# peteroh23/ModulationDetectionCNN

Hardware: AMD Instinct MI355X
Metric: I/Q frames/sec (2x128, VT-CNN2, batch=2^20) (higher is better)
Workload: dtype bf16; 1 GPU; vtcnn2-c11-bf16-n2^20; topology=vtcnn2, classes=11, frames_per_gpu=1048576, global_batch=1048576, parallelism=batch-shard x1 (no collective), outputs=softmax probabilities f32 + argmax int32, frames_per_forward_call=1048576, full=False

## Files before the change

modulationdetectioncnn_amd/build.py:

```python
from __future__ import annotations

import hashlib
import os
import shutil
import subprocess
import sys
from concurrent.futures import ThreadPoolExecutor

HERE = os.path.dirname(os.path.abspath(__file__))
ROOT = os.path.dirname(HERE)
CSRC = os.path.join(HERE, "csrc")
OBJ = os.path.join(HERE, "csrc", "build")
LIB = os.path.join(HERE, "libmdc.so")
ARCH = "gfx950"
VERSION_SCRIPT = os.path.join(CSRC, "libmdc.map")
VARIANTS = {"product": (OBJ, LIB, ()),
            "alternates": (os.path.join(HERE, "csrc", "build_alt"), os.path.join(HERE, "libmdc_alt.so"), ("-DMDC_ALTERNATES",))}

CXXFLAGS = ["-O3", "-std=c++17", "-fPIC", f"--offload-arch={ARCH}", "-I", os.path.join(ROOT, "include"),
            "-I", CSRC, "-Wall", "-Wno-unused-function", "-pthread",
            "-fvisibility=hidden", "-fvisibility-inlines-hidden"]


def _hipcc() -> str:
    exe = shutil.which("hipcc") or "/opt/rocm/bin/hipcc"
    if not os.path.exists(exe):
        raise RuntimeError("hipcc not found: libmdc.so cannot be built")
    return exe


def sources():
    return sorted(os.path.join(CSRC, f) for f in os.listdir(CSRC) if f.endswith(".hip"))


def _newer(a: str, deps) -> bool:
    if not os.path.exists(a):
        return False
    t = os.path.getmtime(a)
    return all(os.path.getmtime(d) <= t for d in deps)


def flag_key(extra_flags=()) -> str:
    return hashlib.sha256(" ".join([*CXXFLAGS, *extra_flags]).encode()).hexdigest()


def build(force: bool = False, verbose: bool = False, extra_flags=(), variant: str = "product") -> str:
    obj_dir, lib_path, vflags = VARIANTS[variant]
    extra_flags = (*vflags, *extra_flags)
    os.makedirs(obj_dir, exist_ok=True)
    stamp = os.path.join(obj_dir, "flags.stamp")
    hipcc = _hipcc()
    headers = [os.path.join(CSRC, f) for f in os.listdir(CSRC) if f.endswith(".h")] + [os.path.join(ROOT, "include", "mdc.h")]
    key = flag_key(extra_flags)
    if not (os.path.exists(stamp) and open(stamp).read().strip() == key):
        force = True
    jobs = []
    objs = []
    for src in sources():
        obj = os.path.join(obj_dir, os.path.basename(src)[:-4] + ".o")
        objs.append(obj)
        if force or not _newer(obj, [src] + headers):
            jobs.append((src, obj))
# ... 39 lines not shown
```

modulationdetectioncnn_amd/csrc/mdc_api.hip:

```cpp
#include "mdc_internal.h"

#include <cstdlib>
#include <cstring>
#include <exception>
#include <mutex>
#include <new>

namespace mdc {

static thread_local char g_err[512] = "";

void set_error(const char* fmt, ...) {
    va_list ap;
    va_start(ap, fmt);
    vsnprintf(g_err, sizeof(g_err), fmt, ap);
    va_end(ap);
}

int upload(mdc_model* m, int idx, const void* host, size_t bytes) {
    if (m->d_pack[idx]) {
        (void)hipFree(m->d_pack[idx]);
        m->d_pack[idx] = nullptr;
    }
    MDC_HIP(hipMalloc(&m->d_pack[idx], bytes));
// ... 96 lines not shown
        if (std::strncmp(prop.gcnArchName, "gfx950", 6) != 0) {
            set_error("device %d is %s; libmdc.so carries gfx950 (MI355X) code only", device, prop.gcnArchName);
            return MDC_ENODEV;
        }
        mdc_model* m = new (std::nothrow) mdc_model();
        if (!m) { set_error("out of host memory"); return MDC_ENOMEM; }
        m->topo = *topo;
        m->device = device;
#ifdef MDC_ALTERNATES
        {
            auto flag = [](const char* name, int when) { const char* e = getenv(name); return e && atoi(e) == when; };
            if (flag("MDC_CONV_SCHED", 0)) m->alt |= kAltConvHipcc;
            if (flag("MDC_DENSE1_PHASED", 0)) m->alt |= kAltDense1Simple;
            if (flag("MDC_DEP_F32_MFMA", 1)) m->alt |= kAltDepF32Mfma;
            if (flag("MDC_D1_FUSED_HEAD", 0)) m->alt |= kAltSeparateHead;
            if (const char* e = getenv("MDC_DEP_RING")) m->alt_ring = atoi(e);
        }
#endif
        int rc = MDC_ENOMEM;
        try { rc = layer_layout(m); } catch (...) { delete m; throw; }
        if (rc != MDC_OK) { delete m; return rc; }
        *out = m;
        return MDC_OK;
    });
}

int mdc_num_layers(const mdc_model* m) {
    if (!m) { set_error("null model"); return MDC_EINVAL; }
    return m->nlayers;
}
// ... 341 lines not shown
```

modulationdetectioncnn_amd/csrc/mdc_internal.h:

```cpp
#pragma once
#include <hip/hip_runtime.h>
#include <cstdarg>
#include <cstdint>
#include <cstdio>
#include <exception>
#include <mutex>
#include <new>
#include <string>
#include <type_traits>
#include <vector>

#include "mdc.h"

namespace mdc {

void set_error(const char* fmt, ...);

template <class Fn>
inline int guarded(const char* what, Fn&& fn) noexcept {
    try {
        return fn();
    } catch (const std::bad_alloc&) {
        set_error("%s: out of host memory", what);
        return MDC_ENOMEM;
// ... 47 lines not shown
};
template <bool CHECK> using HopOrNf = typename std::conditional<CHECK, NfArgs, long>::type;
__device__ __forceinline__ long hop_of(long h) { return h; }
__device__ __forceinline__ long hop_of(const NfArgs&) { return 256; }
__device__ __forceinline__ NfArgs nf_of(long) { return NfArgs{nullptr, nullptr, 0}; }
__device__ __forceinline__ NfArgs nf_of(const NfArgs& a) { return a; }
constexpr unsigned kNfInfBits = 0x7F800000u;
__device__ __forceinline__ unsigned nf_absbits_max4(const float4 v) {
    return max(max(__float_as_uint(v.x) & 0x7FFFFFFFu, __float_as_uint(v.y) & 0x7FFFFFFFu),
               max(__float_as_uint(v.z) & 0x7FFFFFFFu, __float_as_uint(v.w) & 0x7FFFFFFFu));
}

enum { kAltConvHipcc = 1,
       kAltDense1Simple = 2,
       kAltDepF32Mfma = 4,
       kAltSeparateHead = 8 };

struct ProfSlot {
    const char* name;
    std::vector<hipEvent_t> ev;
    double total_ms = 0;
    int64_t launches = 0;
};

}

struct mdc_model {
    mdc_topology topo{};
    int device = 0;
    int dtype = MDC_F32;
    bool finalized = false;
// ... 60 lines not shown
                    int64_t chunk_frames);
int predict_host_iq_norm(mdc_model* m, const void* iq_host, int format, int64_t n, int64_t hop, float level, int flags, float* probs_host,
                         int32_t* labels_host, mdc_iq_window_stats64* stats_host, int64_t chunk_frames);
void host_ctx_free(mdc_model* m);

int deployed_pack(mdc_model* m);
int deployed_f32m_pack(mdc_model* m);
int deployed_f32m_forward(const mdc_model* m, const float* x, int64_t n, float* probs, int32_t* labels, float* tap_dense, hipStream_t s);
int deployed_f32m_forward_iq_u8(const mdc_model* m, const uint8_t* iq, int64_t n, long hop2, float scale, float* probs, int32_t* labels, hipStream_t s);
int deployed_bf16_pack(mdc_model* m);
int deployed_bf16_forward(const mdc_model* m, const float* x, int64_t n, float* probs, int32_t* labels, hipStream_t s);
int deployed_bf16_forward_iq_u8(const mdc_model* m, const uint8_t* iq, int64_t n, int64_t hop, float scale, float* probs, int32_t* labels, hipStream_t s);
int deployed_q612_pack(mdc_model* m);
int deployed_q612_forward(const mdc_model* m, const void* x, int x_is_q, int64_t n, int32_t* dense, int32_t* labels, hipStream_t s);
int vtcnn2_fp8_pack(mdc_model* m);
int vtcnn2_fp8_conv(const mdc_model* m, const float* x, int64_t n, void* feat, hipStream_t s, long hop2 = 0, float scale = 0.f);
int confusion_launch(const int32_t* truth, const int32_t* pred, const int32_t* bin, int64_t n, int classes, int bins, int64_t* counts,
                     int64_t* bad, hipStream_t s);
int crossentropy_launch(const float* probs, const int32_t* truth, int64_t n, int classes, double* loss_sum, int64_t* bad, hipStream_t s);
int iq_u8_launch(const uint8_t* iq, int64_t n, int64_t hop, float scale, float* x, hipStream_t s);
int iq_norm_check(const char* who, int64_t hop, float level, int flags);
int iq_norm_launch(const uint8_t* iq, int64_t n, int64_t hop, float level, int flags, float* x, mdc_iq_window_stats* stats, hipStream_t s);
int iq_pair_bytes(int format);
int iq_format_check(const char* who, int format, int64_t hop);
int iq_fmt_windows_launch(const void* iq, int format, int64_t n, int64_t hop, float scale, float* x, hipStream_t s);
int iq_fmt_norm_launch(const void* iq, int format, int64_t n, int64_t hop, float level, int flags, float* x, mdc_iq_window_stats64* stats,
                       hipStream_t s);
int nonfinite_launch(const float* x, int64_t n, uint8_t* flags, int64_t* count, float* probs, int32_t* labels, int classes, bool poison,
                     hipStream_t s);
int deployed_forward(const mdc_model* m, const float* x, int64_t n, float* probs, int32_t* labels,
                     float* tap, int tap_kind, hipStream_t s);
// ... 19 lines not shown
```

modulationdetectioncnn_amd/csrc/vtcnn2.hip:

```cpp
#include "dense_chain_common.h"

#include <algorithm>
#include <cmath>

namespace mdc {

namespace {

__device__ __forceinline__ void glds16(const void* g, void* lds_wave_base) {
    const unsigned l = (unsigned)(size_t)(__attribute__((address_space(3))) unsigned char*)lds_wave_base;
    asm volatile("global_load_lds_dwordx4 %0, off" ::"v"(g), "{m0}"(l) : "memory");
}
__device__ __forceinline__ void glds_drain_and_barrier() {
    asm volatile("s_waitcnt vmcnt(0)" ::: "memory");
    __syncthreads();
}

constexpr int kChunk = 16;
constexpr int kNChunk = kC1 / kChunk;
constexpr int kWChunkFloats = 2 * 3 * 5 * 4 * 64;
constexpr int kXld = 133;
constexpr int kXinFloats = 4 * 2 * 16 * kXld;
constexpr size_t kConvF32Lds = (2 * kWChunkFloats + kXinFloats) * sizeof(float);

// ... 372 lines not shown
    const int o = r / kW2, w = r % kW2;
    const unsigned v = feat[f * kFeat + feat8_index(w, o)];
    const int e = (int)((v >> 3) & 15u), mant = (int)(v & 7u);
    float mag = e == 0 ? ldexpf((float)mant, -9) : ldexpf(1.f + (float)mant * 0.125f, e - 7);
    if ((v & 0x7Fu) == 0x7Fu) mag = __uint_as_float(0x7FC00000u);
    out[i] = ((v & 0x80u) ? -mag : mag) * unscale;
}

}

void chain_pack_layer(std::vector<float>& dst, const float* w, int k_in, int n_out, int ksteps, int tiles);
int chain_launch(int t1, int nl, const float* x, long n, const float* wpack, int n_out, int relu1, int relu2,
                 float* probs, int* labels, float* tap_logits, float* tap_h1, float* tap_h2, int n1, int n2, hipStream_t s);

int vtcnn2_bf16_pack(mdc_model* m);
int vtcnn2_bf16_conv(const mdc_model* m, const float* x, int64_t n, void* feat, hipStream_t s, long hop2 = 0, float scale = 0.f);
int vtcnn2_bf16_dense1(const mdc_model* m, const void* feat, int64_t n, float* hid, hipStream_t s,
                       bool fuse_head, float* probs, int32_t* labels, bool* fused);

int vtcnn2_pack(mdc_model* m) {
    const float* k1 = m->hk[0].data();
    const float* b1 = m->hb[0].data();
    const float* k2 = m->hk[1].data();
    int rc;
    if ((rc = upload(m, 2, m->hb[1].data(), kC2 * sizeof(float)))) return rc;
    if ((rc = upload(m, 4, m->hb[2].data(), kHid * sizeof(float)))) return rc;
    {
        const int C = m->topo.classes;
        if (C > 16) { set_error("vtcnn2: the HIP head covers up to 16 classes (got %d)", C); return MDC_ENOTSUP; }
        std::vector<float> pk;
        chain_pack_layer(pk, m->hk[3].data(), kHid, C, 64, 1);
// ... 41 lines not shown
    return np * kFeat * feat_elem(m) + np * kHid * sizeof(float);
}

static int vtcnn2_run(const mdc_model* m, const float* x, long hop2, float scale, int64_t n, float* probs, int32_t* labels,
                      float* tap, int tap_kind, void* ws, size_t ws_bytes, hipStream_t s) {
    const size_t need = vtcnn2_workspace_bytes(m, n);
    if (!ws || ws_bytes < need) { set_error("vtcnn2 forward of %lld frames needs %zu workspace bytes (got %zu)", (long long)n, need, ws_bytes); return MDC_EINVAL; }
    if ((reinterpret_cast<uintptr_t>(ws) & 255) != 0) { set_error("workspace must be 256-byte aligned"); return MDC_EINVAL; }
    const size_t fbytes = (((size_t)n + 255) & ~(size_t)255) * kFeat * feat_elem(m);
    void* feat = ws;
    float* hid = reinterpret_cast<float*>(static_cast<char*>(ws) + fbytes);
    const int C = m->topo.classes;
    int rc;
    bool head_done = false;
    if (m->dtype == MDC_BF16 || m->dtype == MDC_FP8) {
        { ProfScope ps(m, 0, s); if ((rc = m->dtype == MDC_FP8 ? vtcnn2_fp8_conv(m, x, n, feat, s, hop2, scale) : vtcnn2_bf16_conv(m, x, n, feat, s, hop2, scale))) return rc; }
        const bool fuse = tap_kind != MDC_TAP_DENSE && tap_kind != MDC_TAP_HIDDEN;
        { ProfScope ps(m, 1, s); if ((rc = vtcnn2_bf16_dense1(m, feat, n, hid, s, fuse, probs, labels, &head_done))) return rc; }
    } else {
        {
            ProfScope ps(m, 0, s);
            const unsigned groups = (unsigned)((n + 63) / 64);
            constexpr long t1 = 128, t3 = 2048, t11 = 8192;
#define MDC_LAUNCH_CONV_F32(U, KP, YS) do { \
                MDC_HIP(hipFuncSetAttribute(reinterpret_cast<const void*>(vt_conv_f32_kernel<U, KP, YS>), hipFuncAttributeMaxDynamicSharedMemorySize, (int)kConvF32Lds)); \
                hipLaunchKernelGGL((vt_conv_f32_kernel<U, KP, YS>), dim3(groups, YS ? kW2 / KP : 1), dim3(256), kConvF32Lds, s, x, (long)n, \
                                   static_cast<const float*>(m->d_pack[0]), static_cast<const float*>(m->d_pack[1]), \
                                   static_cast<const float*>(m->d_pack[2]), static_cast<float*>(feat), hop2 > 0 ? hop2 : 256L, scale); } while (0)
            if (hop2 > 0) {
                if (n <= t1) MDC_LAUNCH_CONV_F32(true, 1, true);
                else if (n <= t3) MDC_LAUNCH_CONV_F32(true, 3, true);
// ... 82 lines not shown
```

modulationdetectioncnn_amd/csrc/vtcnn2_bf16.hip:

```cpp
#include "vtcnn2_bf16_common.h"
#include "vtcnn2_sched_common.h"

#include <cmath>

#include <cstdlib>
#include <cstring>
#include <type_traits>

namespace mdc {

namespace {

#ifdef MDC_ALTERNATES
__global__ __launch_bounds__(256, 1) void vt_conv_bf16_kernel(const float* __restrict__ x, long n,
                                                              const u32x4* __restrict__ wq,
                                                              const u32x2* __restrict__ a1q,
                                                              const float* __restrict__ b2,
                                                              unsigned short* __restrict__ feat) {
    extern __shared__ __attribute__((aligned(16))) unsigned char smem[];
    unsigned* img = reinterpret_cast<unsigned*>(smem);
    float* part = reinterpret_cast<float*>(smem + (size_t)2 * kImgWords * 4);
    const int tid = threadIdx.x, lane = tid & 63;
    const int q = __builtin_amdgcn_readfirstlane(tid >> 6);
    const int nl = lane & 15, g = lane >> 4;
// ... 228 lines not shown
        if ((rc = upload(m, 2, b2s.data(), b2s.size() * sizeof(float)))) return rc;
    }
    m->feat_scale_log2 = -kFeatShift;
    const float* w1 = m->hk[2].data();
    std::vector<unsigned short> w1t((size_t)kHid * kFeat);
    for (int w = 0; w < kW2; ++w)
        for (int o = 0; o < kC2; ++o) {
            const float* src = w1 + (size_t)(o * kW2 + w) * kHid;
            const int kk = feat16_index(w, o);
            for (int nn = 0; nn < kHid; ++nn) w1t[((size_t)(kk >> 6) * kHid + nn) * 64 + (kk & 63)] = f2bf(std::ldexp(src[nn], kFeatShift));
        }
    if ((rc = upload(m, 3, w1t.data(), w1t.size() * 2))) return rc;
    return vtcnn2_bf16_pack_sched(m);
}

int vtcnn2_bf16_conv(const mdc_model* m, const float* x, int64_t n, void* feat, hipStream_t s, long hop2, float scale) {
#ifdef MDC_ALTERNATES
    if ((m->alt & kAltConvHipcc) && hop2 <= 0) {
        const long ngroups = (n + 15) / 16;
        const unsigned grid = (unsigned)(ngroups < 256 ? ngroups : 256);
        MDC_HIP(hipFuncSetAttribute(reinterpret_cast<const void*>(vt_conv_bf16_kernel), hipFuncAttributeMaxDynamicSharedMemorySize, (int)kConvBf16Lds));
        hipLaunchKernelGGL(vt_conv_bf16_kernel, dim3(grid), dim3(256), kConvBf16Lds, s, x, (long)n,
                           static_cast<const u32x4*>(m->d_pack[0]), static_cast<const u32x2*>(m->d_pack[1]),
                           static_cast<const float*>(m->d_pack[2]), static_cast<unsigned short*>(feat));
        MDC_HIP(hipGetLastError());
        return MDC_OK;
    }
#endif
    return vtcnn2_bf16_conv_sched(m, x, n, feat, s, hop2, scale);
}

}
```

modulationdetectioncnn_amd/csrc/vtcnn2_bf16_common.h:

```cpp
#pragma once
#include "mdc_internal.h"

#include <cstring>

namespace mdc {

using f32x4 = __attribute__((ext_vector_type(4))) float;
using f32x2 = __attribute__((ext_vector_type(2))) float;
using bf16x8 = __attribute__((ext_vector_type(8))) __bf16;
using bf16x2 = __attribute__((ext_vector_type(2))) __bf16;
using s16x4 = __attribute__((ext_vector_type(4))) short;
using s16x2 = __attribute__((ext_vector_type(2))) short;
using u32x4 = __attribute__((ext_vector_type(4))) unsigned;
using u32x2 = __attribute__((ext_vector_type(2))) unsigned;

namespace {

constexpr int kPairs = 67;
constexpr int kImgWords = 2 * kPairs * 64;
constexpr int kPartFloats = 4 * 5 * 64 * 4;
constexpr size_t kConvBf16Lds = (size_t)2 * kImgWords * 4 + (size_t)2 * kPartFloats * 4 + 512;
constexpr int kWFrags = 2 * 3 * 2 * 5;

__device__ __forceinline__ unsigned pack2(float a, float b) {
// ... 71 lines not shown
    unsigned u;
    std::memcpy(&u, &f, 4);
    if ((u & 0x7F800000u) == 0x7F800000u) return (unsigned short)(u >> 16);
    u += 0x7FFFu + ((u >> 16) & 1u);
    return (unsigned short)(u >> 16);
}
inline float bf2f(unsigned short h) {
    unsigned u = (unsigned)h << 16;
    float f;
    std::memcpy(&f, &u, 4);
    return f;
}

}

int vtcnn2_bf16_conv_sched(const mdc_model* m, const float* x, int64_t n, void* feat, hipStream_t s, long hop2 = 0, float scale = 0.f);
int vtcnn2_bf16_pack_sched(mdc_model* m);

}
```

modulationdetectioncnn_amd/csrc/vtcnn2_bf16_sched.hip:

```cpp
#include "vtcnn2_bf16_common.h"
#include "vtcnn2_sched_common.h"

#include <cmath>
#include <cstdlib>
#include <type_traits>

namespace mdc {

namespace {

constexpr int kNV = 24;

struct SchedState {
    u32x4 Wv[kNV];
    u32x4 Wa[kWFrags - kNV];
    f32x4 bias[5];
    u32x4 A1[2];
    unsigned Bf[2][2][2][4];
    f32x16 X[2];
    f32x4 rp[4];
    float rc[4];
    float tprev;
    u32x4 L0[3];
    u32x4 L1;
// ... 123 lines not shown
#undef FIN
#undef PREP
#undef C1M
#undef ST
#undef WR
#undef PK
#undef RD
#undef LD
#undef HANDOFF
}

template <int ABL, bool U8 = false, bool RANGE = false>
__global__ __launch_bounds__(256, 1) void vt_conv_bf16_sched_kernel(const float* __restrict__ x, long n,
                                                                    const u32x4* __restrict__ wq, const u32x4* __restrict__ a1q,
                                                                    const float* __restrict__ b2, unsigned short* __restrict__ feat,
                                                                    long hop2 = 256, float scale = 0.f) {
    extern __shared__ __attribute__((aligned(16))) unsigned char smem[];
    unsigned* img = reinterpret_cast<unsigned*>(smem);
    const int tid = threadIdx.x, lane = tid & 63;
    const int q = __builtin_amdgcn_readfirstlane(tid >> 6);
    const int nl = lane & 15, g = lane >> 4;

    SchedState st;
#pragma unroll
    for (int i = 0; i < kWFrags; ++i) {
        const u32x4 w = wq[(q * kWFrags + i) * 64 + lane];
        if (i < kNV) { st.Wv[i] = w; asm volatile("" : "+v"(st.Wv[i])); }
        else { st.Wa[i - kNV] = w; asm volatile("" : "+a"(st.Wa[i - kNV])); }
    }
    st.A1[0] = a1q[(q * 2 + 0) * 64 + lane];
    st.A1[1] = a1q[(q * 2 + 1) * 64 + lane];
#pragma unroll
// ... 18 lines not shown
    st.cb[0] = st.cb[1] = st.cb[2] = st.cb[3] = 0u;
    st.tprev = 0.f;

    for (int i = tid; i < 2 * kSImgWords; i += 256) img[i] = ((((i / kS) & 63) >= 32) && ((i % kS) & 1)) ? 0x3F803F80u : 0u;
    __syncthreads();
    const long ngroups = (n + 15) >> 4;
    long grp = blockIdx.x;
    if (grp < ngroups)
        for (int k = 0; k < 4; ++k) sch_stage_write(k, stage_decode<U8>(stage_load<U8>(k, x, n, grp * 16, tid, hop2), tid, scale), n, grp * 16, img, tid);
    __syncthreads();
    const int rng = RANGE ? (int)blockIdx.y : 0;
    const int S = 12 * rng;
    const int wlo = rng ? S + 2 : 0;

    int buf = 0;
    for (; grp < ngroups; grp += gridDim.x, buf ^= 1) {
        st.im_addr = img_lds + (buf * kSImgWords + lane * kS) * 4;
        unsigned short* fbase = feat + (grp * 16 + fs) * (long)(kW2 * kC2);
        const long gnext = RANGE ? ngroups : grp + gridDim.x;
        f32x4 acc[3][5];
        {
            const u32x4 zero = u32x4{0u, 0u, 0u, 0u};
#pragma unroll
            for (int b = 0; b < 5; ++b) {
                asm volatile("s_nop 1\n\tv_mfma_f32_16x16x32_bf16 %0, %1, %1, %2" : "=&a"(acc[0][b]) : "v"(zero), "a"(st.bias[b]));
                asm volatile("v_mfma_f32_16x16x32_bf16 %0, %1, %1, %2" : "=&a"(acc[1][b]) : "v"(zero), "a"(st.bias[b]));
            }
        }

        sch_load_even<0>(st, st.im_addr + (S >> 2) * 16);
        sch_load_odd(st, st.im_addr + (S >> 2) * 16 + 8);
        sch_wait_lds(st);
        sch_conv1_mfma<0, 0, 0>(st); sch_conv1_mfma<0, 0, 1>(st);
        asm volatile("s_nop 7\n\ts_nop 7\n\ts_nop 7\n\ts_nop 7\n\ts_nop 7\n\ts_nop 7\n\ts_nop 7\n\ts_nop 7" : "+v"(st.X[0]), "+v"(st.X[1]));
        [&]<int... N>(std::integer_sequence<int, N...>) { (sch_packop<0, N>(st), ...); }(std::make_integer_sequence<int, 16>{});
        asm volatile("s_nop 1");

        sch_step<0, true, false, ABL, RANGE>(st, S, q, fbase, acc, wlo);
        const int iters = RANGE ? (rng < 10 ? 1 : 0) : 10;
        int v = S + 1;
        typename StageRaw<U8>::type sv{};
        for (int it = 0; it < iters; ++it, v += 12) {
            if constexpr (!RANGE) {
                if (it >= 6 && gnext < ngroups) sch_stage_write(it - 6, stage_decode<U8>(sv, tid, scale), n, gnext * 16, img + (buf ^ 1) * kSImgWords, tid);
                if (it >= 5 && it < 9 && gnext < ngroups) sv = stage_load<U8>(it - 5, x, n, gnext * 16, tid, hop2);
            }
            sch_step<1, false, false, ABL, RANGE>(st, v + 0, q, fbase, acc, wlo);
            sch_step<2, false, false, ABL, RANGE>(st, v + 1, q, fbase, acc, wlo);
            sch_step<3, false, false, ABL, RANGE>(st, v + 2, q, fbase, acc, wlo);
            sch_step<4, false, false, ABL, RANGE>(st, v + 3, q, fbase, acc, wlo);
            sch_step<5, false, false, ABL, RANGE>(st, v + 4, q, fbase, acc, wlo);
            sch_step<6, false, false, ABL, RANGE>(st, v + 5, q, fbase, acc, wlo);
            sch_step<7, false, false, ABL, RANGE>(st, v + 6, q, fbase, acc, wlo);
            sch_step<8, false, false, ABL, RANGE>(st, v + 7, q, fbase, acc, wlo);
            sch_step<9, false, false, ABL, RANGE>(st, v + 8, q, fbase, acc, wlo);
            sch_step<10, false, false, ABL, RANGE>(st, v + 9, q, fbase, acc, wlo);
            sch_step<11, false, false, ABL, RANGE>(st, v + 10, q, fbase, acc, wlo);
            sch_step<0, false, false, ABL, RANGE>(st, v + 11, q, fbase, acc, wlo);
        }
        const int vt = RANGE ? v : 121;
// ... 31 lines not shown
        asm volatile("s_nop 7\n\ts_nop 7");
        sch_part_write<0, 0>(st, acc[1][0]); sch_part_write<0, 1>(st, acc[1][1]); sch_part_write<0, 2>(st, acc[1][2]);
        sch_part_write<0, 3>(st, acc[1][3]); sch_part_write<0, 4>(st, acc[1][4]);
        asm volatile("s_waitcnt lgkmcnt(0)\n\ts_barrier" ::: "memory");
        sch_red_load<0>(st);
        asm volatile("" ::"a"(acc[1][0]), "a"(acc[1][1]), "a"(acc[1][2]), "a"(acc[1][3]), "a"(acc[1][4]));
        finish_store(Even{}, 130);
        sch_part_write<1, 0>(st, acc[2][0]); sch_part_write<1, 1>(st, acc[2][1]); sch_part_write<1, 2>(st, acc[2][2]);
        sch_part_write<1, 3>(st, acc[2][3]); sch_part_write<1, 4>(st, acc[2][4]);
        asm volatile("s_waitcnt lgkmcnt(0)\n\ts_barrier" ::: "memory");
        sch_red_load<1>(st);
        asm volatile("" ::"a"(acc[2][0]), "a"(acc[2][1]), "a"(acc[2][2]), "a"(acc[2][3]), "a"(acc[2][4]));
        finish_store(Odd{}, 131);
        __syncthreads();
    }
}

}

int vtcnn2_bf16_pack_sched(mdc_model* m) {
    const float* k1 = m->hk[0].data();
    const float* b1 = m->hb[0].data();
    const float* k2 = m->hk[1].data();
    int rc;
    std::vector<unsigned short> wq((size_t)4 * kWFrags * 64 * 8);
    for (int q = 0; q < 4; ++q)
        for (int ct = 0; ct < 2; ++ct)
            for (int j = 0; j < 3; ++j)
                for (int bb = 0; bb < 2; ++bb)
                    for (int ot = 0; ot < 5; ++ot)
// ... 15 lines not shown
                unsigned short th[3], tl[3];
                for (int t = 0; t < 3; ++t) {
                    th[t] = f2bf(k1[ch * 3 + t] * sc);
                    tl[t] = f2bf(k1[ch * 3 + t] * sc - bf2f(th[t]));
                }
                if (khalf == 0) {
                    d[0] = th[0]; d[1] = th[1]; d[2] = th[0]; d[3] = th[1]; d[4] = th[2]; d[6] = th[2];
                } else {
                    const unsigned short bh = f2bf(b1[ch] * sc);
                    d[0] = tl[0]; d[1] = tl[1]; d[2] = bh; d[3] = f2bf(b1[ch] * sc - bf2f(bh)); d[4] = tl[2];
                }
            }
    return upload(m, 7, a1.data(), a1.size() * 2);
}

int vtcnn2_bf16_conv_sched(const mdc_model* m, const float* x, int64_t n, void* feat, hipStream_t s, long hop2, float scale) {
    const long ngroups = (n + 15) / 16;
    const unsigned grid = (unsigned)(ngroups < 256 ? ngroups : 256);
#define MDC_LAUNCH_SCHED_V(U, R, GRID) do { \
    MDC_HIP(hipFuncSetAttribute(reinterpret_cast<const void*>(vt_conv_bf16_sched_kernel<0, U, R>), hipFuncAttributeMaxDynamicSharedMemorySize, (int)kSchedLds)); \
    hipLaunchKernelGGL((vt_conv_bf16_sched_kernel<0, U, R>), GRID, dim3(256), kSchedLds, s, x, (long)n, \
                       static_cast<const u32x4*>(m->d_pack[6]), static_cast<const u32x4*>(m->d_pack[7]), \
                       static_cast<const float*>(m->d_pack[2]), static_cast<unsigned short*>(feat), hop2 > 0 ? hop2 : 256L, scale); \
    MDC_HIP(hipGetLastError()); return MDC_OK; } while (0)
    if (n <= kConvRangeFrames) {
        if (hop2 > 0) MDC_LAUNCH_SCHED_V(true, true, dim3((unsigned)ngroups, 11));
        else MDC_LAUNCH_SCHED_V(false, true, dim3((unsigned)ngroups, 11));
    }
    if (hop2 > 0) MDC_LAUNCH_SCHED_V(true, false, dim3(grid));
#undef MDC_LAUNCH_SCHED_V
#define MDC_LAUNCH_SCHED(A) do { \
    MDC_HIP(hipFuncSetAttribute(reinterpret_cast<const void*>(vt_conv_bf16_sched_kernel<A>), hipFuncAttributeMaxDynamicSharedMemorySize, (int)kSchedLds)); \
    hipLaunchKernelGGL(vt_conv_bf16_sched_kernel<A>, dim3(grid), dim3(256), kSchedLds, s, x, (long)n, \
                       static_cast<const u32x4*>(m->d_pack[6]), static_cast<const u32x4*>(m->d_pack[7]), \
                       static_cast<const float*>(m->d_pack[2]), static_cast<unsigned short*>(feat), 256L, 0.f); } while (0)
#ifdef MDC_ABLATIONS
    static const int abl = getenv("MDC_ABLATE_S") ? atoi(getenv("MDC_ABLATE_S")) : 0;
    switch (abl) { case 1: MDC_LAUNCH_SCHED(1); break; case 2: MDC_LAUNCH_SCHED(2); break; case 3: MDC_LAUNCH_SCHED(3); break;
                   case 5: MDC_LAUNCH_SCHED(5); break; case 6: MDC_LAUNCH_SCHED(6); break; case 7: MDC_LAUNCH_SCHED(7); break;
                   case 8: MDC_LAUNCH_SCHED(8); break; case 9: MDC_LAUNCH_SCHED(9); break; case 10: MDC_LAUNCH_SCHED(10); break;
                   case 11: MDC_LAUNCH_SCHED(11); break; default: MDC_LAUNCH_SCHED(0); }
#else
    MDC_LAUNCH_SCHED(0);
#endif
#undef MDC_LAUNCH_SCHED
    MDC_HIP(hipGetLastError());
    return MDC_OK;
}

}
// ... 1 lines not shown
```

modulationdetectioncnn_amd/csrc/vtcnn2_fp8_conv.hip:

```cpp
#include "vtcnn2_bf16_common.h"
#include "vtcnn2_sched_common.h"

#include <cmath>
#include <cstdlib>

namespace mdc {

namespace {

using u32x8 = __attribute__((ext_vector_type(8))) unsigned;
constexpr int kF8Frags = 15;
constexpr int kF8NV = 7;

struct Fp8State {
    u32x8 Wv[kF8NV];
    u32x8 Wa[kF8Frags - kF8NV];
    f32x4 bias[5];
    u32x4 A1[2];
    unsigned Bf[2][8];
    unsigned one;
    unsigned scb;
    float sc9;
    f32x16 X[2];
    unsigned T[16];
// ... 135 lines not shown
#undef PREP
#undef C1M
#undef ST
#undef WR
#undef PKB
#undef CV
#undef RD
#undef LD
#undef HANDOFF
}

template <bool U8, bool RANGE = false, bool F8OUT = true>
__global__ __launch_bounds__(256, 1) void vt_conv_fp8_kernel(const float* __restrict__ x, long n,
                                                             const u32x8* __restrict__ wq, const u32x4* __restrict__ a1q,
                                                             const float* __restrict__ b2, void* __restrict__ feat_out,
                                                             long hop2, float scale, unsigned scale_b_e8m0, float feat_divisor) {
    using FeatT = typename std::conditional<F8OUT, unsigned char, unsigned short>::type;
    FeatT* __restrict__ feat = static_cast<FeatT*>(feat_out);
    extern __shared__ __attribute__((aligned(16))) unsigned char smem[];
    unsigned* img = reinterpret_cast<unsigned*>(smem);
    const int tid = threadIdx.x, lane = tid & 63;
    const int q = __builtin_amdgcn_readfirstlane(tid >> 6);
    const int nl = lane & 15, g = lane >> 4;

    Fp8State st;
#pragma unroll
    for (int i = 0; i < kF8Frags; ++i) {
        const u32x8 w = wq[(q * kF8Frags + i) * 64 + lane];
        if (i < kF8NV) { st.Wv[i] = w; asm volatile("" : "+v"(st.Wv[i])); }
        else { st.Wa[i - kF8NV] = w; asm volatile("" : "+a"(st.Wa[i - kF8NV])); }
    }
    st.A1[0] = a1q[(q * 2 + 0) * 64 + lane];
    st.A1[1] = a1q[(q * 2 + 1) * 64 + lane];
    asm volatile("s_setreg_imm32_b32 hwreg(HW_REG_MODE, 23, 1), 1");
// ... 29 lines not shown
#pragma unroll
    for (int d = 0; d < 8; ++d) st.Bf[0][d] = st.Bf[1][d] = 0u;

    for (int i = tid; i < 2 * kSImgWords; i += 256) img[i] = ((((i / kS) & 63) >= 32) && ((i % kS) & 1)) ? 0x3F803F80u : 0u;
    __syncthreads();
    const long ngroups = (n + 15) >> 4;
    long grp = blockIdx.x;
    if (grp < ngroups)
        for (int k = 0; k < 4; ++k) sch_stage_write(k, stage_decode<U8>(stage_load<U8>(k, x, n, grp * 16, tid, hop2), tid, scale), n, grp * 16, img, tid);
    __syncthreads();
    const int rng = RANGE ? (int)blockIdx.y : 0;
    const int S = 12 * rng;
    const int wlo = rng ? S + 2 : 0;

    int buf = 0;
    for (; grp < ngroups; grp += gridDim.x, buf ^= 1) {
        st.im_addr = img_lds + (buf * kSImgWords + lane * kS) * 4;
        FeatT* fbase = feat + (grp * 16 + fs) * (long)(kW2 * kC2);
        const long gnext = RANGE ? ngroups : grp + gridDim.x;
        f32x4 acc[3][5];
        {
            const u32x4 zero = u32x4{0u, 0u, 0u, 0u};
#pragma unroll
            for (int b = 0; b < 5; ++b) {
                asm volatile("s_nop 1\n\tv_mfma_f32_16x16x32_bf16 %0, %1, %1, %2" : "=&a"(acc[0][b]) : "v"(zero), "a"(st.bias[b]));
                asm volatile("v_mfma_f32_16x16x32_bf16 %0, %1, %1, %2" : "=&a"(acc[1][b]) : "v"(zero), "a"(st.bias[b]));
            }
        }
        sch_load_even<0>(st, st.im_addr + (S >> 2) * 16);
        sch_load_odd(st, st.im_addr + (S >> 2) * 16 + 8);
        sch_wait_lds(st);
        sch_conv1_mfma<0, 0, 0>(st); sch_conv1_mfma<0, 0, 1>(st);
        asm volatile("s_nop 7\n\ts_nop 7\n\ts_nop 7\n\ts_nop 7\n\ts_nop 7\n\ts_nop 7\n\ts_nop 7\n\ts_nop 7" : "+v"(st.X[0]), "+v"(st.X[1]));
        [&]<int... K>(std::integer_sequence<int, K...>) { (f8_pkb<K>(st), ...); }(std::make_integer_sequence<int, 16>{});
        [&]<int... K>(std::integer_sequence<int, K...>) { (f8_cvt<0, K>(st), ...); }(std::make_integer_sequence<int, 16>{});
        asm volatile("s_nop 1");

        f8_step<0, true, false, RANGE, F8OUT>(st, S, q, fbase, acc, wlo);
        const int iters = RANGE ? (rng < 10 ? 1 : 0) : 10;
        int v = S + 1;
        typename StageRaw<U8>::type sv{};
        for (int it = 0; it < iters; ++it, v += 12) {
            if constexpr (!RANGE) {
                if (it >= 6 && gnext < ngroups) sch_stage_write(it - 6, stage_decode<U8>(sv, tid, scale), n, gnext * 16, img + (buf ^ 1) * kSImgWords, tid);
                if (it >= 5 && it < 9 && gnext < ngroups) sv = stage_load<U8>(it - 5, x, n, gnext * 16, tid, hop2);
            }
            f8_step<1, false, false, RANGE, F8OUT>(st, v + 0, q, fbase, acc, wlo);
            f8_step<2, false, false, RANGE, F8OUT>(st, v + 1, q, fbase, acc, wlo);
            f8_step<3, false, false, RANGE, F8OUT>(st, v + 2, q, fbase, acc, wlo);
            f8_step<4, false, false, RANGE, F8OUT>(st, v + 3, q, fbase, acc, wlo);
            f8_step<5, false, false, RANGE, F8OUT>(st, v + 4, q, fbase, acc, wlo);
            f8_step<6, false, false, RANGE, F8OUT>(st, v + 5, q, fbase, acc, wlo);
            f8_step<7, false, false, RANGE, F8OUT>(st, v + 6, q, fbase, acc, wlo);
            f8_step<8, false, false, RANGE, F8OUT>(st, v + 7, q, fbase, acc, wlo);
            f8_step<9, false, false, RANGE, F8OUT>(st, v + 8, q, fbase, acc, wlo);
            f8_step<10, false, false, RANGE, F8OUT>(st, v + 9, q, fbase, acc, wlo);
            f8_step<11, false, false, RANGE, F8OUT>(st, v + 10, q, fbase, acc, wlo);
            f8_step<0, false, false, RANGE, F8OUT>(st, v + 11, q, fbase, acc, wlo);
        }
        const int vt = RANGE ? v : 121;
// ... 45 lines not shown
        asm volatile("s_nop 7\n\ts_nop 7");
        sch_part_write<0, 0>(st, acc[1][0]); sch_part_write<0, 1>(st, acc[1][1]); sch_part_write<0, 2>(st, acc[1][2]);
        sch_part_write<0, 3>(st, acc[1][3]); sch_part_write<0, 4>(st, acc[1][4]);
        asm volatile("s_waitcnt lgkmcnt(0)\n\ts_barrier" ::: "memory");
        sch_red_load<0>(st);
        asm volatile("" ::"a"(acc[1][0]), "a"(acc[1][1]), "a"(acc[1][2]), "a"(acc[1][3]), "a"(acc[1][4]));
        finish_store(Even{}, 130);
        sch_part_write<1, 0>(st, acc[2][0]); sch_part_write<1, 1>(st, acc[2][1]); sch_part_write<1, 2>(st, acc[2][2]);
        sch_part_write<1, 3>(st, acc[2][3]); sch_part_write<1, 4>(st, acc[2][4]);
        asm volatile("s_waitcnt lgkmcnt(0)\n\ts_barrier" ::: "memory");
        sch_red_load<1>(st);
        asm volatile("" ::"a"(acc[2][0]), "a"(acc[2][1]), "a"(acc[2][2]), "a"(acc[2][3]), "a"(acc[2][4]));
        finish_store(Last{}, 131);
        __syncthreads();
    }
}

}

static unsigned char f2e4m3(float f) {
    if (std::isnan(f)) return 0x7F;
    const unsigned char sign = std::signbit(f) ? 0x80 : 0x00;
    float a = std::fabs(f);
    if (a >= 448.f) return sign | 0x7E;
    if (a < std::ldexp(1.f, -10)) return sign;
    int e;
    (void)std::frexp(a, &e);
    int E = e - 1;
    if (E < -6) E = -6;
    const float q = std::nearbyint(std::ldexp(a, 3 - E));
// ... 83 lines not shown
        m->feat_scale_log2 = kf;
        m->fp8_feat_divisor = std::ldexp(1.f, -(kFeatShift + kf));
    }
    const float* w1 = m->hk[2].data();
    const float inv = std::ldexp(1.f, m->fp8_e4m3_features ? -kf : kFeatShift);
    std::vector<unsigned short> w1t((size_t)kHid * kFeat);
    for (int w = 0; w < kW2; ++w)
        for (int o = 0; o < kC2; ++o) {
            const float* srcw = w1 + (size_t)(o * kW2 + w) * kHid;
            const int kk = m->fp8_e4m3_features ? feat8_index(w, o) : feat16_index(w, o);
            for (int nn = 0; nn < kHid; ++nn) w1t[((size_t)(kk >> 6) * kHid + nn) * 64 + (kk & 63)] = f2bf(srcw[nn] * inv);
        }
    return upload(m, 3, w1t.data(), w1t.size() * 2);
}

int vtcnn2_fp8_conv(const mdc_model* m, const float* x, int64_t n, void* feat, hipStream_t s, long hop2, float scale) {
    const long ngroups = (n + 15) / 16;
    const unsigned grid = (unsigned)(ngroups < 256 ? ngroups : 256);
#define MDC_LAUNCH_F8(U, R, F, GRID) do { \
    MDC_HIP(hipFuncSetAttribute(reinterpret_cast<const void*>(vt_conv_fp8_kernel<U, R, F>), hipFuncAttributeMaxDynamicSharedMemorySize, (int)kSchedLds)); \
    hipLaunchKernelGGL((vt_conv_fp8_kernel<U, R, F>), GRID, dim3(256), kSchedLds, s, x, (long)n, \
                       static_cast<const u32x8*>(m->d_pack[0]), static_cast<const u32x4*>(m->d_pack[1]), \
                       static_cast<const float*>(m->d_pack[2]), feat, hop2 > 0 ? hop2 : 256L, scale, \
                       (unsigned)m->fp8_feat_scale_log2, m->fp8_feat_divisor); } while (0)
#define MDC_LAUNCH_F8_UR(U, R, GRID) do { if (m->fp8_e4m3_features) MDC_LAUNCH_F8(U, R, true, GRID); else MDC_LAUNCH_F8(U, R, false, GRID); } while (0)
    if (n <= kConvRangeFrames) {
        if (hop2 > 0) MDC_LAUNCH_F8_UR(true, true, dim3((unsigned)ngroups, 11));
        else MDC_LAUNCH_F8_UR(false, true, dim3((unsigned)ngroups, 11));
    } else {
        if (hop2 > 0) MDC_LAUNCH_F8_UR(true, false, dim3(grid));
        else MDC_LAUNCH_F8_UR(false, false, dim3(grid));
    }
#undef MDC_LAUNCH_F8_UR
#undef MDC_LAUNCH_F8
    MDC_HIP(hipGetLastError());
    return MDC_OK;
}

}
// ... 1 lines not shown
```

modulationdetectioncnn_amd/csrc/vtcnn2_sched_common.h:

```cpp
#pragma once
#include "vtcnn2_bf16_common.h"

#include <type_traits>
#include <utility>

namespace mdc {

namespace {

constexpr int kS = 140;
constexpr int kSImgWords = 64 * kS;
constexpr long kConvRangeFrames = 1024;
constexpr size_t kSchedLds = (size_t)2 * kSImgWords * 4 + (size_t)2 * kPartFloats * 4;

using f32x16 = __attribute__((ext_vector_type(16))) float;

template <int SLOT, class S>
__device__ __forceinline__ void sch_load_even(S& st, unsigned entry_addr) {
    asm volatile("ds_read_b128 %0, %1" : "=v"(st.L0[SLOT]) : "v"(entry_addr) : "memory");
}
template <class S>
__device__ __forceinline__ void sch_load_odd(S& st, unsigned entry_addr) {
    asm volatile("ds_read2_b64 %0, %1 offset0:0 offset1:1" : "=v"(st.L1) : "v"(entry_addr) : "memory");
}
template <int R, int S0, int SN, int I, class S>
__device__ __forceinline__ void sch_prep(S& st) {
    if constexpr (R == 1 || R == 3) {
        const unsigned w0 = R == 1 ? st.L0[S0][0] : st.L1[0], w1 = R == 1 ? st.L0[S0][1] : st.L1[1];
        const unsigned w2 = R == 1 ? st.L0[S0][2] : st.L1[2], w3 = R == 1 ? st.L0[S0][3] : st.L1[3];
        const unsigned w4 = R == 1 ? st.L1[2] : st.L0[SN][2], w5 = R == 1 ? st.L1[3] : st.L0[SN][3];
// ... 50 lines not shown
    } else if constexpr (ODD) asm volatile("v_cvt_pk_bf16_f32 %0, %1, %2 clamp" : "=v"(out.tt) : "v"(st.tprev), "v"(f.t));
}
template <int ODD, class S>
__device__ __forceinline__ void sch_fin_all_clamp(S& st, FinOut& out) {
    FinTmp f;
    [&]<int... K>(std::integer_sequence<int, K...>) { (sch_fin_clamp<K, ODD>(st, f, out), ...); }(std::make_integer_sequence<int, 18>{});
}

template <int WHICH>
__device__ __forceinline__ void sch_store(const FinOut& fo, unsigned short* frow, int w, int q, int gs) {
    unsigned short* pair = frow + (long)(w >> 1) * (2 * kC2);
    if constexpr (WHICH == 0) *reinterpret_cast<u32x2*>(pair + (w & 1) * 64 + 16 * q + 4 * gs) = u32x2{fo.o0, fo.o1};
    else *reinterpret_cast<unsigned*>(pair + 128 + 2 * (4 * q + gs)) = fo.tt;
}

__device__ __forceinline__ void sch_stage_write(int k, float4 v, long n, long frame0, unsigned* __restrict__ im, int tid) {
    const int idx = tid + 256 * k;
    const int i = idx >> 6, l = idx & 63;
    if (frame0 + i >= n) v = make_float4(0.f, 0.f, 0.f, 0.f);
    const int h = l >> 5, m = l & 31;
    const float xs[4] = {v.x, v.y, v.z, v.w};
#pragma unroll
    for (int e = 0; e < 2; ++e) {
        const float a = xs[2 * e], b = xs[2 * e + 1];
        const unsigned hi = pack2(a, b);
        const float ah = __uint_as_float(hi << 16), bh = __uint_as_float(hi & 0xFFFF0000u);
        const unsigned lo = pack2(a - ah, b - bh);
        unsigned* d = im + (i + 16 * h) * kS + 2 * (2 * m + 1 + e);
        *reinterpret_cast<u32x2*>(d) = u32x2{hi, lo};
        d[32 * kS] = hi;
// ... 8 lines not shown
```

Measured before the change: 41.91 million frames/s.

## Replace static grid-stride group assignment in conv kernels with atomic ticket scheduling

The persistent conv kernels (bf16 and fp8) now claim their next 16-frame group from a global atomic counter instead of striding by gridDim.x. Each block draws a ticket a few passes before it needs the group and publishes it through LDS so the prefetch of the next group's input still overlaps compute. The counter borrows the hidden-activation buffer and is zeroed with a memset before launch. The aim is to balance load across blocks and XCDs when some finish faster, at the cost of one atomic per group, an extra memset, and an added register pin on the staged input. Timestamp probes and a build variant for ablations are also added.

Result: no change. 42.33 million frames/s, median of 6 (+1.0%).

```diff
diff --git a/modulationdetectioncnn_amd/build.py b/modulationdetectioncnn_amd/build.py
--- a/modulationdetectioncnn_amd/build.py
+++ b/modulationdetectioncnn_amd/build.py
@@ -16,6 +16,7 @@
 VERSION_SCRIPT = os.path.join(CSRC, "libmdc.map")
 VARIANTS = {"product": (OBJ, LIB, ()),
             "alternates": (os.path.join(HERE, "csrc", "build_alt"), os.path.join(HERE, "libmdc_alt.so"), ("-DMDC_ALTERNATES",))}
+PROBES = {"probes": (os.path.join(HERE, "csrc", "build_probe"), os.path.join(HERE, "libmdc_probe.so"), ("-DMDC_ALTERNATES", "-DMDC_ABLATIONS"))}
 
 CXXFLAGS = ["-O3", "-std=c++17", "-fPIC", f"--offload-arch={ARCH}", "-I", os.path.join(ROOT, "include"),
             "-I", CSRC, "-Wall", "-Wno-unused-function", "-pthread",
@@ -45,7 +46,7 @@
 
 
 def build(force: bool = False, verbose: bool = False, extra_flags=(), variant: str = "product") -> str:
-    obj_dir, lib_path, vflags = VARIANTS[variant]
+    obj_dir, lib_path, vflags = {**VARIANTS, **PROBES}[variant]
     extra_flags = (*vflags, *extra_flags)
     os.makedirs(obj_dir, exist_ok=True)
     stamp = os.path.join(obj_dir, "flags.stamp")
diff --git a/modulationdetectioncnn_amd/csrc/mdc_api.hip b/modulationdetectioncnn_amd/csrc/mdc_api.hip
--- a/modulationdetectioncnn_amd/csrc/mdc_api.hip
+++ b/modulationdetectioncnn_amd/csrc/mdc_api.hip
@@ -134,6 +134,7 @@
             if (flag("MDC_DENSE1_PHASED", 0)) m->alt |= kAltDense1Simple;
             if (flag("MDC_DEP_F32_MFMA", 1)) m->alt |= kAltDepF32Mfma;
             if (flag("MDC_D1_FUSED_HEAD", 0)) m->alt |= kAltSeparateHead;
+            if (flag("MDC_CONV_TICKETS", 0)) m->alt |= kAltConvStride;
             if (const char* e = getenv("MDC_DEP_RING")) m->alt_ring = atoi(e);
         }
 #endif
diff --git a/modulationdetectioncnn_amd/csrc/mdc_internal.h b/modulationdetectioncnn_amd/csrc/mdc_internal.h
--- a/modulationdetectioncnn_amd/csrc/mdc_internal.h
+++ b/modulationdetectioncnn_amd/csrc/mdc_internal.h
@@ -85,7 +85,8 @@
 enum { kAltConvHipcc = 1,
        kAltDense1Simple = 2,
        kAltDepF32Mfma = 4,
-       kAltSeparateHead = 8 };
+       kAltSeparateHead = 8,
+       kAltConvStride = 16 };
 
 struct ProfSlot {
     const char* name;
@@ -176,7 +177,7 @@
 int deployed_q612_pack(mdc_model* m);
 int deployed_q612_forward(const mdc_model* m, const void* x, int x_is_q, int64_t n, int32_t* dense, int32_t* labels, hipStream_t s);
 int vtcnn2_fp8_pack(mdc_model* m);
-int vtcnn2_fp8_conv(const mdc_model* m, const float* x, int64_t n, void* feat, hipStream_t s, long hop2 = 0, float scale = 0.f);
+int vtcnn2_fp8_conv(const mdc_model* m, const float* x, int64_t n, void* feat, hipStream_t s, long hop2 = 0, float scale = 0.f, unsigned* counter = nullptr);
 int confusion_launch(const int32_t* truth, const int32_t* pred, const int32_t* bin, int64_t n, int classes, int bins, int64_t* counts,
                      int64_t* bad, hipStream_t s);
 int crossentropy_launch(const float* probs, const int32_t* truth, int64_t n, int classes, double* loss_sum, int64_t* bad, hipStream_t s);
diff --git a/modulationdetectioncnn_amd/csrc/vtcnn2.hip b/modulationdetectioncnn_amd/csrc/vtcnn2.hip
--- a/modulationdetectioncnn_amd/csrc/vtcnn2.hip
+++ b/modulationdetectioncnn_amd/csrc/vtcnn2.hip
@@ -410,7 +410,7 @@
                  float* probs, int* labels, float* tap_logits, float* tap_h1, float* tap_h2, int n1, int n2, hipStream_t s);
 
 int vtcnn2_bf16_pack(mdc_model* m);
-int vtcnn2_bf16_conv(const mdc_model* m, const float* x, int64_t n, void* feat, hipStream_t s, long hop2 = 0, float scale = 0.f);
+int vtcnn2_bf16_conv(const mdc_model* m, const float* x, int64_t n, void* feat, hipStream_t s, long hop2 = 0, float scale = 0.f, unsigned* counter = nullptr);
 int vtcnn2_bf16_dense1(const mdc_model* m, const void* feat, int64_t n, float* hid, hipStream_t s,
                        bool fuse_head, float* probs, int32_t* labels, bool* fused);
 
@@ -482,7 +482,8 @@
     int rc;
     bool head_done = false;
     if (m->dtype == MDC_BF16 || m->dtype == MDC_FP8) {
-        { ProfScope ps(m, 0, s); if ((rc = m->dtype == MDC_FP8 ? vtcnn2_fp8_conv(m, x, n, feat, s, hop2, scale) : vtcnn2_bf16_conv(m, x, n, feat, s, hop2, scale))) return rc; }
+        unsigned* counter = reinterpret_cast<unsigned*>(hid);
+        { ProfScope ps(m, 0, s); if ((rc = m->dtype == MDC_FP8 ? vtcnn2_fp8_conv(m, x, n, feat, s, hop2, scale, counter) : vtcnn2_bf16_conv(m, x, n, feat, s, hop2, scale, counter))) return rc; }
         const bool fuse = tap_kind != MDC_TAP_DENSE && tap_kind != MDC_TAP_HIDDEN;
         { ProfScope ps(m, 1, s); if ((rc = vtcnn2_bf16_dense1(m, feat, n, hid, s, fuse, probs, labels, &head_done))) return rc; }
     } else {
diff --git a/modulationdetectioncnn_amd/csrc/vtcnn2_bf16.hip b/modulationdetectioncnn_amd/csrc/vtcnn2_bf16.hip
--- a/modulationdetectioncnn_amd/csrc/vtcnn2_bf16.hip
+++ b/modulationdetectioncnn_amd/csrc/vtcnn2_bf16.hip
@@ -266,7 +266,7 @@
     return vtcnn2_bf16_pack_sched(m);
 }
 
-int vtcnn2_bf16_conv(const mdc_model* m, const float* x, int64_t n, void* feat, hipStream_t s, long hop2, float scale) {
+int vtcnn2_bf16_conv(const mdc_model* m, const float* x, int64_t n, void* feat, hipStream_t s, long hop2, float scale, unsigned* counter) {
 #ifdef MDC_ALTERNATES
     if ((m->alt & kAltConvHipcc) && hop2 <= 0) {
         const long ngroups = (n + 15) / 16;
@@ -279,7 +279,7 @@
         return MDC_OK;
     }
 #endif
-    return vtcnn2_bf16_conv_sched(m, x, n, feat, s, hop2, scale);
-}
-
-}
+    return vtcnn2_bf16_conv_sched(m, x, n, feat, s, hop2, scale, counter);
+}
+
+}
diff --git a/modulationdetectioncnn_amd/csrc/vtcnn2_bf16_common.h b/modulationdetectioncnn_amd/csrc/vtcnn2_bf16_common.h
--- a/modulationdetectioncnn_amd/csrc/vtcnn2_bf16_common.h
+++ b/modulationdetectioncnn_amd/csrc/vtcnn2_bf16_common.h
@@ -109,7 +109,8 @@
 
 }
 
-int vtcnn2_bf16_conv_sched(const mdc_model* m, const float* x, int64_t n, void* feat, hipStream_t s, long hop2 = 0, float scale = 0.f);
+int vtcnn2_bf16_conv_sched(const mdc_model* m, const float* x, int64_t n, void* feat, hipStream_t s, long hop2 = 0, float scale = 0.f,
+                           unsigned* counter = nullptr);
 int vtcnn2_bf16_pack_sched(mdc_model* m);
 
 }
diff --git a/modulationdetectioncnn_amd/csrc/vtcnn2_bf16_sched.hip b/modulationdetectioncnn_amd/csrc/vtcnn2_bf16_sched.hip
--- a/modulationdetectioncnn_amd/csrc/vtcnn2_bf16_sched.hip
+++ b/modulationdetectioncnn_amd/csrc/vtcnn2_bf16_sched.hip
@@ -161,8 +161,14 @@
 __global__ __launch_bounds__(256, 1) void vt_conv_bf16_sched_kernel(const float* __restrict__ x, long n,
                                                                     const u32x4* __restrict__ wq, const u32x4* __restrict__ a1q,
                                                                     const float* __restrict__ b2, unsigned short* __restrict__ feat,
-                                                                    long hop2 = 256, float scale = 0.f) {
+                                                                    long hop2 = 256, float scale = 0.f,
+                                                                    unsigned* ticket = nullptr MDC_STAMP_PARAM) {
     extern __shared__ __attribute__((aligned(16))) unsigned char smem[];
+    __shared__ unsigned tk_lds[2];
+#ifdef MDC_ABLATIONS
+    sch_stamp_entry(stamps);
+    int groups_done = 0;
+#endif
     unsigned* img = reinterpret_cast<unsigned*>(smem);
     const int tid = threadIdx.x, lane = tid & 63;
     const int q = __builtin_amdgcn_readfirstlane(tid >> 6);
@@ -211,10 +217,15 @@
     const int wlo = rng ? S + 2 : 0;
 
     int buf = 0;
-    for (; grp < ngroups; grp += gridDim.x, buf ^= 1) {
+    long gnext = ngroups;
+    unsigned tk = 0;
+    for (; grp < ngroups; grp = RANGE ? grp + gridDim.x : gnext, buf ^= 1) {
         st.im_addr = img_lds + (buf * kSImgWords + lane * kS) * 4;
         unsigned short* fbase = feat + (grp * 16 + fs) * (long)(kW2 * kC2);
-        const long gnext = RANGE ? ngroups : grp + gridDim.x;
+        gnext = RANGE ? ngroups : grp + gridDim.x;
+#ifdef MDC_ABLATIONS
+        ++groups_done;
+#endif
         f32x4 acc[3][5];
         {
             const u32x4 zero = u32x4{0u, 0u, 0u, 0u};
@@ -239,8 +250,13 @@
         typename StageRaw<U8>::type sv{};
         for (int it = 0; it < iters; ++it, v += 12) {
             if constexpr (!RANGE) {
-                if (it >= 6 && gnext < ngroups) sch_stage_write(it - 6, stage_decode<U8>(sv, tid, scale), n, gnext * 16, img + (buf ^ 1) * kSImgWords, tid);
+                if (ticket && it == 5) gnext = (long)(unsigned)__builtin_amdgcn_readfirstlane((int)tk_lds[buf]);
+                if (it >= 6 && gnext < ngroups) { sch_stage_pin(sv); sch_stage_write(it - 6, stage_decode<U8>(sv, tid, scale), n, gnext * 16, img + (buf ^ 1) * kSImgWords, tid); }
                 if (it >= 5 && it < 9 && gnext < ngroups) sv = stage_load<U8>(it - 5, x, n, gnext * 16, tid, hop2);
+                if (ticket && tid == 0) {
+                    if (it == kTicketDrawPass) tk = sch_ticket_draw(ticket);
+                    else if (it == kTicketDrawPass + 1) tk_lds[buf] = gridDim.x + tk;
+                }
             }
             sch_step<1, false, false, ABL, RANGE>(st, v + 0, q, fbase, acc, wlo);
             sch_step<2, false, false, ABL, RANGE>(st, v + 1, q, fbase, acc, wlo);
@@ -302,6 +318,9 @@
         finish_store(Odd{}, 131);
         __syncthreads();
     }
+#ifdef MDC_ABLATIONS
+    sch_stamp_exit(stamps, groups_done);
+#endif
 }
 
 }
@@ -347,14 +366,20 @@
     return upload(m, 7, a1.data(), a1.size() * 2);
 }
 
-int vtcnn2_bf16_conv_sched(const mdc_model* m, const float* x, int64_t n, void* feat, hipStream_t s, long hop2, float scale) {
+int vtcnn2_bf16_conv_sched(const mdc_model* m, const float* x, int64_t n, void* feat, hipStream_t s, long hop2, float scale, unsigned* counter) {
     const long ngroups = (n + 15) / 16;
     const unsigned grid = (unsigned)(ngroups < 256 ? ngroups : 256);
+    unsigned* ticket = nullptr;
+    if (int rc = conv_ticket_prepare(m, n, ngroups, grid, counter, s, &ticket)) return rc;
+#ifdef MDC_ABLATIONS
+    unsigned long long* stamps = conv_stamp_records(counter);
+#endif
 #define MDC_LAUNCH_SCHED_V(U, R, GRID) do { \
     MDC_HIP(hipFuncSetAttribute(reinterpret_cast<const void*>(vt_conv_bf16_sched_kernel<0, U, R>), hipFuncAttributeMaxDynamicSharedMemorySize, (int)kSchedLds)); \
     hipLaunchKernelGGL((vt_conv_bf16_sched_kernel<0, U, R>), GRID, dim3(256), kSchedLds, s, x, (long)n, \
                        static_cast<const u32x4*>(m->d_pack[6]), static_cast<const u32x4*>(m->d_pack[7]), \
-                       static_cast<const float*>(m->d_pack[2]), static_cast<unsigned short*>(feat), hop2 > 0 ? hop2 : 256L, scale); \
+                       static_cast<const float*>(m->d_pack[2]), static_cast<unsigned short*>(feat), hop2 > 0 ? hop2 : 256L, scale, \
+                       R ? nullptr : ticket MDC_STAMP_ARG(stamps)); \
     MDC_HIP(hipGetLastError()); return MDC_OK; } while (0)
     if (n <= kConvRangeFrames) {
         if (hop2 > 0) MDC_LAUNCH_SCHED_V(true, true, dim3((unsigned)ngroups, 11));
@@ -366,7 +391,7 @@
     MDC_HIP(hipFuncSetAttribute(reinterpret_cast<const void*>(vt_conv_bf16_sched_kernel<A>), hipFuncAttributeMaxDynamicSharedMemorySize, (int)kSchedLds)); \
     hipLaunchKernelGGL(vt_conv_bf16_sched_kernel<A>, dim3(grid), dim3(256), kSchedLds, s, x, (long)n, \
                        static_cast<const u32x4*>(m->d_pack[6]), static_cast<const u32x4*>(m->d_pack[7]), \
-                       static_cast<const float*>(m->d_pack[2]), static_cast<unsigned short*>(feat), 256L, 0.f); } while (0)
+                       static_cast<const float*>(m->d_pack[2]), static_cast<unsigned short*>(feat), 256L, 0.f, ticket MDC_STAMP_ARG(stamps)); } while (0)
 #ifdef MDC_ABLATIONS
     static const int abl = getenv("MDC_ABLATE_S") ? atoi(getenv("MDC_ABLATE_S")) : 0;
     switch (abl) { case 1: MDC_LAUNCH_SCHED(1); break; case 2: MDC_LAUNCH_SCHED(2); break; case 3: MDC_LAUNCH_SCHED(3); break;
diff --git a/modulationdetectioncnn_amd/csrc/vtcnn2_fp8_conv.hip b/modulationdetectioncnn_amd/csrc/vtcnn2_fp8_conv.hip
--- a/modulationdetectioncnn_amd/csrc/vtcnn2_fp8_conv.hip
+++ b/modulationdetectioncnn_amd/csrc/vtcnn2_fp8_conv.hip
@@ -173,10 +173,16 @@
 __global__ __launch_bounds__(256, 1) void vt_conv_fp8_kernel(const float* __restrict__ x, long n,
                                                              const u32x8* __restrict__ wq, const u32x4* __restrict__ a1q,
                                                              const float* __restrict__ b2, void* __restrict__ feat_out,
-                                                             long hop2, float scale, unsigned scale_b_e8m0, float feat_divisor) {
+                                                             long hop2, float scale, unsigned scale_b_e8m0, float feat_divisor,
+                                                             unsigned* ticket = nullptr MDC_STAMP_PARAM) {
     using FeatT = typename std::conditional<F8OUT, unsigned char, unsigned short>::type;
     FeatT* __restrict__ feat = static_cast<FeatT*>(feat_out);
     extern __shared__ __attribute__((aligned(16))) unsigned char smem[];
+    __shared__ unsigned tk_lds[2];
+#ifdef MDC_ABLATIONS
+    sch_stamp_entry(stamps);
+    int groups_done = 0;
+#endif
     unsigned* img = reinterpret_cast<unsigned*>(smem);
     const int tid = threadIdx.x, lane = tid & 63;
     const int q = __builtin_amdgcn_readfirstlane(tid >> 6);
@@ -236,10 +242,15 @@
     const int wlo = rng ? S + 2 : 0;
 
     int buf = 0;
-    for (; grp < ngroups; grp += gridDim.x, buf ^= 1) {
+    long gnext = ngroups;
+    unsigned tk = 0;
+    for (; grp < ngroups; grp = RANGE ? grp + gridDim.x : gnext, buf ^= 1) {
         st.im_addr = img_lds + (buf * kSImgWords + lane * kS) * 4;
         FeatT* fbase = feat + (grp * 16 + fs) * (long)(kW2 * kC2);
-        const long gnext = RANGE ? ngroups : grp + gridDim.x;
+        gnext = RANGE ? ngroups : grp + gridDim.x;
+#ifdef MDC_ABLATIONS
+        ++groups_done;
+#endif
         f32x4 acc[3][5];
         {
             const u32x4 zero = u32x4{0u, 0u, 0u, 0u};
@@ -264,8 +275,13 @@
         typename StageRaw<U8>::type sv{};
         for (int it = 0; it < iters; ++it, v += 12) {
             if constexpr (!RANGE) {
-                if (it >= 6 && gnext < ngroups) sch_stage_write(it - 6, stage_decode<U8>(sv, tid, scale), n, gnext * 16, img + (buf ^ 1) * kSImgWords, tid);
+                if (ticket && it == 5) gnext = (long)(unsigned)__builtin_amdgcn_readfirstlane((int)tk_lds[buf]);
+                if (it >= 6 && gnext < ngroups) { sch_stage_pin(sv); sch_stage_write(it - 6, stage_decode<U8>(sv, tid, scale), n, gnext * 16, img + (buf ^ 1) * kSImgWords, tid); }
                 if (it >= 5 && it < 9 && gnext < ngroups) sv = stage_load<U8>(it - 5, x, n, gnext * 16, tid, hop2);
+                if (ticket && tid == 0) {
+                    if (it == kTicketDrawPass) tk = sch_ticket_draw(ticket);
+                    else if (it == kTicketDrawPass + 1) tk_lds[buf] = gridDim.x + tk;
+                }
             }
             f8_step<1, false, false, RANGE, F8OUT>(st, v + 0, q, fbase, acc, wlo);
             f8_step<2, false, false, RANGE, F8OUT>(st, v + 1, q, fbase, acc, wlo);
@@ -341,6 +357,9 @@
         finish_store(Last{}, 131);
         __syncthreads();
     }
+#ifdef MDC_ABLATIONS
+    sch_stamp_exit(stamps, groups_done);
+#endif
 }
 
 }
@@ -454,15 +473,20 @@
     return upload(m, 3, w1t.data(), w1t.size() * 2);
 }
 
-int vtcnn2_fp8_conv(const mdc_model* m, const float* x, int64_t n, void* feat, hipStream_t s, long hop2, float scale) {
+int vtcnn2_fp8_conv(const mdc_model* m, const float* x, int64_t n, void* feat, hipStream_t s, long hop2, float scale, unsigned* counter) {
     const long ngroups = (n + 15) / 16;
     const unsigned grid = (unsigned)(ngroups < 256 ? ngroups : 256);
+    unsigned* ticket = nullptr;
+    if (int rc = conv_ticket_prepare(m, n, ngroups, grid, counter, s, &ticket)) return rc;
+#ifdef MDC_ABLATIONS
+    unsigned long long* stamps = conv_stamp_records(counter);
+#endif
 #define MDC_LAUNCH_F8(U, R, F, GRID) do { \
     MDC_HIP(hipFuncSetAttribute(reinterpret_cast<const void*>(vt_conv_fp8_kernel<U, R, F>), hipFuncAttributeMaxDynamicSharedMemorySize, (int)kSchedLds)); \
     hipLaunchKernelGGL((vt_conv_fp8_kernel<U, R, F>), GRID, dim3(256), kSchedLds, s, x, (long)n, \
                        static_cast<const u32x8*>(m->d_pack[0]), static_cast<const u32x4*>(m->d_pack[1]), \
                        static_cast<const float*>(m->d_pack[2]), feat, hop2 > 0 ? hop2 : 256L, scale, \
-                       (unsigned)m->fp8_feat_scale_log2, m->fp8_feat_divisor); } while (0)
+                       (unsigned)m->fp8_feat_scale_log2, m->fp8_feat_divisor, R ? nullptr : ticket MDC_STAMP_ARG(stamps)); } while (0)
 #define MDC_LAUNCH_F8_UR(U, R, GRID) do { if (m->fp8_e4m3_features) MDC_LAUNCH_F8(U, R, true, GRID); else MDC_LAUNCH_F8(U, R, false, GRID); } while (0)
     if (n <= kConvRangeFrames) {
         if (hop2 > 0) MDC_LAUNCH_F8_UR(true, true, dim3((unsigned)ngroups, 11));
diff --git a/modulationdetectioncnn_amd/csrc/vtcnn2_sched_common.h b/modulationdetectioncnn_amd/csrc/vtcnn2_sched_common.h
--- a/modulationdetectioncnn_amd/csrc/vtcnn2_sched_common.h
+++ b/modulationdetectioncnn_amd/csrc/vtcnn2_sched_common.h
@@ -1,6 +1,7 @@
 #pragma once
 #include "vtcnn2_bf16_common.h"
 
+#include <cstdlib>
 #include <type_traits>
 #include <utility>
 
@@ -14,6 +15,53 @@
 constexpr size_t kSchedLds = (size_t)2 * kSImgWords * 4 + (size_t)2 * kPartFloats * 4;
 
 using f32x16 = __attribute__((ext_vector_type(16))) float;
+
+constexpr int kTicketDrawPass = 3;
+constexpr long kTicketMaxGroups = 0xFFFFFFFFL - 512;
+__device__ __forceinline__ unsigned sch_ticket_draw(unsigned* ticket) {
+    auto* g = (__attribute__((address_space(1))) unsigned*)ticket;
+    asm volatile("" : "+v"(g));
+    return __hip_atomic_fetch_add(g, 1u, __ATOMIC_RELAXED, __HIP_MEMORY_SCOPE_AGENT);
+}
+
+inline int conv_ticket_prepare(const mdc_model* m, int64_t n, long ngroups, unsigned grid, unsigned* counter, hipStream_t s, unsigned** ticket) {
+    *ticket = nullptr;
+    if (!counter || n <= kConvRangeFrames || ngroups <= (long)grid) return MDC_OK;
+#ifdef MDC_ALTERNATES
+    if (m->alt & kAltConvStride) return MDC_OK;
+#endif
+    if (ngroups > kTicketMaxGroups) { set_error("vtcnn2 conv: %ld frame groups do not fit the 32-bit group counter", ngroups); return MDC_EINVAL; }
+    MDC_HIP(hipMemsetAsync(counter, 0, sizeof(unsigned), s));
+    *ticket = counter;
+    return MDC_OK;
+}
+
+constexpr size_t kStampOffsetBytes = 256;
+#ifdef MDC_ABLATIONS
+#define MDC_STAMP_PARAM , unsigned long long* stamps = nullptr
+#define MDC_STAMP_ARG(P) , P
+inline unsigned long long* conv_stamp_records(unsigned* counter) {
+    static const bool on = getenv("MDC_CONV_STAMPS") && atoi(getenv("MDC_CONV_STAMPS")) == 1;
+    return on && counter ? reinterpret_cast<unsigned long long*>(reinterpret_cast<char*>(counter) + kStampOffsetBytes) : nullptr;
+}
+__device__ __forceinline__ void sch_stamp_entry(unsigned long long* stamps) {
+    if (stamps && threadIdx.x == 0) {
+        unsigned xcc;
+        asm volatile("s_getreg_b32 %0, hwreg(HW_REG_XCC_ID, 0, 4)" : "=s"(xcc));
+        stamps[4 * blockIdx.x + 0] = xcc;
+        stamps[4 * blockIdx.x + 1] = wall_clock64();
+    }
+}
+__device__ __forceinline__ void sch_stamp_exit(unsigned long long* stamps, int groups_done) {
+    if (stamps && threadIdx.x == 0) {
+        stamps[4 * blockIdx.x + 2] = wall_clock64();
+        stamps[4 * blockIdx.x + 3] = (unsigned long long)groups_done;
+    }
+}
+#else
+#define MDC_STAMP_PARAM
+#define MDC_STAMP_ARG(P)
+#endif
 
 template <int SLOT, class S>
 __device__ __forceinline__ void sch_load_even(S& st, unsigned entry_addr) {
@@ -94,6 +142,17 @@
     else *reinterpret_cast<unsigned*>(pair + 128 + 2 * (4 * q + gs)) = fo.tt;
 }
 
+__device__ __forceinline__ void sch_stage_pin(float4& v) {
+    f32x4 t = f32x4{v.x, v.y, v.z, v.w};
+    asm volatile("" : "+v"(t));
+    v = make_float4(t[0], t[1], t[2], t[3]);
+}
+__device__ __forceinline__ void sch_stage_pin(uint2& v) {
+    u32x2 t = u32x2{v.x, v.y};
+    asm volatile("" : "+v"(t));
+    v = make_uint2(t[0], t[1]);
+}
+
 __device__ __forceinline__ void sch_stage_write(int k, float4 v, long n, long frame0, unsigned* __restrict__ im, int tid) {
     const int idx = tid + 256 * k;
     const int i = idx >> 6, l = idx & 63;
```
